# george-gca/sr-pytorch-lightning

Hardware: AMD Instinct MI355X
Metric: SR training throughput, LR patches/s (48x48 LR x4, fwd+bwd+Adam) (higher is better)
Workload: dtype bf16; 1 GPU; edsr_baseline x4, 48x48 LR patches, batch 256/GPU, train step (L1 + Adam); global_batch=256, parallelism=dp1, hip_graph=full

## Files before the change

### include/srk.h

```cpp
#ifndef SRK_H
#define SRK_H

#include <stdint.h>

#ifdef __cplusplus
extern "C" {
#endif

typedef void* srk_stream_t;

enum { SRK_BF16 = 0, SRK_F16 = 1, SRK_F32 = 2 };

enum {
  SRK_E_BADARG = -1,
  SRK_E_NODEV = -2
};

enum {
  SRK_OUT_NHWC = 0,
  SRK_OUT_NHWC_PS = 1,
  SRK_OUT_PLANAR = 2
};

typedef struct {
// ... 171 lines not shown
} srk_unfold_args;
int srk_unfold_nchw(const srk_unfold_args* a, srk_stream_t stream);

typedef struct {
  const float* src; void* dst; int dst_pitch, dst_coff;
  int N, C, H, W;
  int Cstore; int ps_r; float scale; int dtype;
} srk_to_nhwc_args;
int srk_nchw_to_nhwc(const srk_to_nhwc_args* a, srk_stream_t stream);

typedef struct {
  const void* src; int src_pitch, src_coff; float* dst;
  int N, C, H, W; int dtype;
} srk_to_nchw_args;
int srk_nhwc_to_nchw(const srk_to_nchw_args* a, srk_stream_t stream);

int srk_ca_splits(int N, int HW);
typedef struct {
  const void* t; int t_pitch, t_coff;
  const void* u; int u_pitch, u_coff;
  float* sums;
  int N, HW, C; int dtype;
} srk_ca_pool_args;
int srk_ca_pool(const srk_ca_pool_args* a, srk_stream_t stream);

typedef struct {
  const void* t; int t_pitch, t_coff;
  const void* res; int res_pitch, res_coff;
  const float* sums;
  const float* w1; const float* b1; const float* w2; const float* b2;
  float* s_out; float* z_out;
  void* out; int out_pitch, out_coff;
  int N, HW, C, Cr; int dtype;
  int sums_rows;
} srk_ca_apply_args;
int srk_ca_apply(const srk_ca_apply_args* a, srk_stream_t stream);

typedef struct {
  const void* g; int g_pitch, g_coff;
  const float* gsum;
  const float* sums; const float* s; const float* z;
  const float* w1; const float* w2;
  float* dw1; float* db1; float* dw2; float* db2;
  void* gt; int gt_pitch, gt_coff;
  int N, HW, C, Cr; int dtype;
  int sums_rows, gsum_rows;
} srk_ca_bwd_args;
int srk_ca_bwd_apply(const srk_ca_bwd_args* a, srk_stream_t stream);
typedef struct { const float* src; float* dst; int n; int k; } srk_rowsum_job;
int srk_rowsum_group(const srk_rowsum_job* table_dev, int njobs, int max_k, srk_stream_t stream);

typedef struct {
  const uint8_t* lr; const uint8_t* hr;
  int lr_h, lr_w, hr_h, hr_w;
  int top, left;
  int rot;
  int hflip, vflip;
} srk_patch_desc;
typedef struct {
  const srk_patch_desc* table; int N; int C; int patch_lr; int scale;
  float* lr_out;
  float* hr_out;
} srk_patch_args;
int srk_sample_patches(const srk_patch_args* a, srk_stream_t stream);

typedef struct {
  const float* sr; const float* hr;
  int N, C, H, W;
  int luma;
  int shave;
  double* sse;
} srk_sse_args;
int srk_image_sse(const srk_sse_args* a, srk_stream_t stream);

typedef struct srk_l1_args {
  const float* sr;
  const float* hr;
  long long n;
  signed char* sign;
  double* partial;
  const float* gout;
  float scale;
  float* grad;
} srk_l1_args;
int srk_l1_blocks(long long n);
int srk_l1_loss_fwd(const srk_l1_args* a, srk_stream_t stream);
int srk_l1_loss_bwd(const srk_l1_args* a, srk_stream_t stream);
int srk_l1_loss_mean(const double* partial, int nb, long long n, float* out, srk_stream_t stream);

#define SRK_FLIP_TABLE_FLOATS 176
#define SRK_FLIP_ADJ_CHANNELS 7
typedef struct srk_flip_args {
  const float* sr;
  const float* hr;
  int N, H, W;
  const float* table;
  double* partial;
  float* err;
  float* adj;
  const float* gout;
  float scale;
  float* grad;
} srk_flip_args;
int srk_flip_blocks(int N, int H, int W);
int srk_flip_fwd(const srk_flip_args* a, srk_stream_t stream);
int srk_flip_bwd(const srk_flip_args* a, srk_stream_t stream);
int srk_flip_mean(const double* partial, int nb, long long n, float* out, srk_stream_t stream);

typedef struct srk_haarpsi_args {
  const float* sr;
  const float* hr;
  int N, C, H, W;
  double* partial;
  float* planes;
  float* stats;
  float* loss;
  float* index;
  const float* gout;
  float* grad;
} srk_haarpsi_args;
int srk_haarpsi_tiles(int N, int H, int W);
int srk_haarpsi_fwd(const srk_haarpsi_args* a, srk_stream_t stream);
int srk_haarpsi_finalize(const srk_haarpsi_args* a, srk_stream_t stream);
int srk_haarpsi_bwd(const srk_haarpsi_args* a, srk_stream_t stream);

typedef struct srk_ssim_args {
  const float* x;
  const float* y;
  int N, C, H, W;
  int pool;
  float sigma, k1, k2;
  double* sums;
} srk_ssim_args;
int srk_image_ssim(const srk_ssim_args* a, srk_stream_t stream);

typedef struct srk_ms_ssim_args {
  const float* x;
  const float* y;
  float* workspace;
  double* partials;
  float* out;
  int N, C, H, W;
  float sigma, k1, k2;
  float w0, w1, w2, w3, w4;
} srk_ms_ssim_args;
long long srk_ms_ssim_workspace_bytes(int N, int C, int H, int W);
int srk_ms_ssim_tiles(int H, int W, int* first);
int srk_ms_ssim(const srk_ms_ssim_args* a, srk_stream_t stream);

typedef struct {
  const void* x; int x_pitch, x_coff;
  void* cols; int cols_pitch;
  int N, H, W, C;
  int K, stride, pad;
  int Ho, Wo;
  int dtype;
} srk_unfold_nhwc_args;
int srk_unfold_nhwc(const srk_unfold_nhwc_args* a, srk_stream_t stream);

typedef struct {
  const void* cols; int cols_pitch;
  const float* bias;
  void* out; int out_pitch, out_coff;
  int N, Hi, Wi, C;
  int K, stride, pad;
  int Ho, Wo;
  int dtype;
} srk_fold_nhwc_args;
int srk_fold_nhwc(const srk_fold_nhwc_args* a, srk_stream_t stream);

// ... 160 lines not shown
```

### sr-pytorch-lightning_amd/_lib.py

```python
import ctypes as C
import os

_HERE = os.path.dirname(os.path.abspath(__file__))
EXACT_RELU = os.environ.get("SRK_EXACT_RELU") == "1"
LIB_PATH = os.environ.get("SRK_LIB_PATH") or os.path.join(_HERE, "libsrk_gfx950_exact.so" if EXACT_RELU else "libsrk_gfx950.so")

SRK_BF16, SRK_F16, SRK_F32 = 0, 1, 2
OUT_NHWC, OUT_NHWC_PS, OUT_PLANAR = 0, 1, 2

_p, _i, _f = C.c_void_p, C.c_int, C.c_float


class PackArgs(C.Structure):
    _fields_ = [("w", _p), ("bias", _p), ("wpk", _p), ("bias_pk", _p),
                ("Cout", _i), ("Cin", _i), ("KH", _i), ("KW", _i),
                ("KinP", _i), ("CoutP", _i), ("dgrad", _i), ("ps_r", _i), ("dtype", _i), ("rows_layout", _i)]


class ConvArgs(C.Structure):
    _fields_ = [("x", _p), ("x_pitch", _i), ("x_coff", _i), ("x_ps", _i),
                ("N", _i), ("H", _i), ("W", _i), ("Cin", _i),
                ("wpk", _p), ("bias", _p), ("CoutP", _i), ("Cout", _i), ("KH", _i), ("KW", _i),
                ("relu", _i), ("scale", _f),
                ("res", _p), ("res_pitch", _i), ("res_coff", _i),
# ... 96 lines not shown
                ("N", _i), ("H", _i), ("W", _i), ("Cin", _i), ("Cout", _i), ("KH", _i), ("KW", _i),
                ("dwp", _p), ("dbp", _p), ("nslabs", _i), ("dtype", _i), ("cout_real", _i)]


class WgradFinArgs(C.Structure):
    _fields_ = [("dwp", _p), ("dbp", _p), ("nslabs", _i), ("dw", _p), ("db", _p),
                ("Cout", _i), ("Cin", _i), ("KH", _i), ("KW", _i), ("CinP", _i), ("CoutP", _i),
                ("ps_r", _i), ("scale", _f), ("accumulate", _i)]


class ProjArgs(C.Structure):
    _fields_ = [("x", _p), ("x_pitch", _i), ("out", _p), ("out_pitch", _i), ("wpk", _p), ("bias", _p),
                ("N", _i), ("H", _i), ("W", _i), ("dtype", _i), ("slope", _p), ("slope_stride", _i), ("pre", _p), ("pre_pitch", _i)]


class ProjPackJob(C.Structure):
    _fields_ = [("w4", _p), ("wpk", _p)]


class ProjWgradArgs(C.Structure):
    _fields_ = [("xh", _p), ("xh_pitch", _i), ("g", _p), ("g_pitch", _i), ("scratch", _p), ("dw", _p), ("accumulate", _i),
                ("N", _i), ("H", _i), ("W", _i), ("dtype", _i), ("db", _p), ("bias_side", _i), ("db_accumulate", _i)]


class UnfoldArgs(C.Structure):
    _fields_ = [("x", _p), ("sub", _p), ("dst", _p), ("dst_pitch", _i), ("dst_coff", _i),
                ("N", _i), ("Cin", _i), ("H", _i), ("W", _i), ("KH", _i), ("KW", _i), ("Kstore", _i), ("dtype", _i)]


class ToNhwcArgs(C.Structure):
    _fields_ = [("src", _p), ("dst", _p), ("dst_pitch", _i), ("dst_coff", _i),
                ("N", _i), ("C", _i), ("H", _i), ("W", _i), ("Cstore", _i), ("ps_r", _i), ("scale", _f), ("dtype", _i)]


class ToNchwArgs(C.Structure):
    _fields_ = [("src", _p), ("src_pitch", _i), ("src_coff", _i), ("dst", _p),
                ("N", _i), ("C", _i), ("H", _i), ("W", _i), ("dtype", _i)]


class CaPoolArgs(C.Structure):
    _fields_ = [("t", _p), ("t_pitch", _i), ("t_coff", _i), ("u", _p), ("u_pitch", _i), ("u_coff", _i),
                ("sums", _p), ("N", _i), ("HW", _i), ("C", _i), ("dtype", _i)]


class CaApplyArgs(C.Structure):
    _fields_ = [("t", _p), ("t_pitch", _i), ("t_coff", _i), ("res", _p), ("res_pitch", _i), ("res_coff", _i),
                ("sums", _p), ("w1", _p), ("b1", _p), ("w2", _p), ("b2", _p), ("s_out", _p), ("z_out", _p),
                ("out", _p), ("out_pitch", _i), ("out_coff", _i),
                ("N", _i), ("HW", _i), ("C", _i), ("Cr", _i), ("dtype", _i), ("sums_rows", _i)]


class CaBwdArgs(C.Structure):
    _fields_ = [("g", _p), ("g_pitch", _i), ("g_coff", _i), ("gsum", _p), ("sums", _p), ("s", _p), ("z", _p),
                ("w1", _p), ("w2", _p), ("dw1", _p), ("db1", _p), ("dw2", _p), ("db2", _p),
                ("gt", _p), ("gt_pitch", _i), ("gt_coff", _i),
                ("N", _i), ("HW", _i), ("C", _i), ("Cr", _i), ("dtype", _i), ("sums_rows", _i), ("gsum_rows", _i)]


class PatchDesc(C.Structure):
    _fields_ = [("lr", _p), ("hr", _p), ("lr_h", _i), ("lr_w", _i), ("hr_h", _i), ("hr_w", _i),
                ("top", _i), ("left", _i), ("rot", _i), ("hflip", _i), ("vflip", _i)]


class PatchArgs(C.Structure):
    _fields_ = [("table", _p), ("N", _i), ("C", _i), ("patch_lr", _i), ("scale", _i), ("lr_out", _p), ("hr_out", _p)]


class SseArgs(C.Structure):
    _fields_ = [("sr", _p), ("hr", _p), ("N", _i), ("C", _i), ("H", _i), ("W", _i), ("luma", _i), ("shave", _i), ("sse", _p)]


class SsimArgs(C.Structure):
    _fields_ = [("x", _p), ("y", _p), ("N", _i), ("C", _i), ("H", _i), ("W", _i), ("pool", _i),
                ("sigma", _f), ("k1", _f), ("k2", _f), ("sums", _p)]


class MsSsimArgs(C.Structure):
    _fields_ = [("x", _p), ("y", _p), ("workspace", _p), ("partials", _p), ("out", _p), ("N", _i), ("C", _i), ("H", _i), ("W", _i),
                ("sigma", _f), ("k1", _f), ("k2", _f), ("w0", _f), ("w1", _f), ("w2", _f), ("w3", _f), ("w4", _f)]


class L1Args(C.Structure):
    _fields_ = [("sr", _p), ("hr", _p), ("n", C.c_longlong), ("sign", _p), ("partial", _p), ("gout", _p),
                ("scale", _f), ("grad", _p)]


class FlipArgs(C.Structure):
    _fields_ = [("sr", _p), ("hr", _p), ("N", _i), ("H", _i), ("W", _i), ("table", _p), ("partial", _p), ("err", _p), ("adj", _p),
                ("gout", _p), ("scale", _f), ("grad", _p)]


class HaarpsiArgs(C.Structure):
    _fields_ = [("sr", _p), ("hr", _p), ("N", _i), ("C", _i), ("H", _i), ("W", _i), ("partial", _p), ("planes", _p), ("stats", _p), ("loss", _p),
                ("index", _p), ("gout", _p), ("grad", _p)]


class UnfoldNhwcArgs(C.Structure):
    _fields_ = [("x", _p), ("x_pitch", _i), ("x_coff", _i), ("cols", _p), ("cols_pitch", _i),
                ("N", _i), ("H", _i), ("W", _i), ("C", _i), ("K", _i), ("stride", _i), ("pad", _i), ("Ho", _i), ("Wo", _i), ("dtype", _i)]


class FoldNhwcArgs(C.Structure):
    _fields_ = [("cols", _p), ("cols_pitch", _i), ("bias", _p), ("out", _p), ("out_pitch", _i), ("out_coff", _i),
                ("N", _i), ("Hi", _i), ("Wi", _i), ("C", _i), ("K", _i), ("stride", _i), ("pad", _i), ("Ho", _i), ("Wo", _i), ("dtype", _i)]


class ChanStatsArgs(C.Structure):
    _fields_ = [("x", _p), ("x_pitch", _i), ("x_coff", _i), ("y", _p), ("y_pitch", _i), ("y_coff", _i),
                ("P", C.c_longlong), ("C", _i), ("mode", _i), ("partial", _p), ("dtype", _i), ("shift", _p), ("shift_out", _p),
                ("gate_out", _p), ("gate_pitch", _i), ("slope", _p), ("slope_stride", _i),
                ("gate_a", _p), ("gate_d", _p), ("partial2", _p)]


class ChanApplyArgs(C.Structure):
    _fields_ = [("x", _p), ("x_pitch", _i), ("x_coff", _i), ("y", _p), ("y_pitch", _i), ("y_coff", _i),
                ("z", _p), ("z_pitch", _i), ("z_coff", _i), ("a", _p), ("b", _p), ("d", _p),
                ("slope", _p), ("slope_stride", _i), ("post_prelu", _i), ("out", _p), ("out_pitch", _i), ("out_coff", _i),
                ("P", C.c_longlong), ("C", _i), ("dtype", _i), ("gate_a", _p), ("gate_d", _p)]


class HrTailArgs(C.Structure):
    _fields_ = [("wt", _p), ("bt", _p), ("wu", _p), ("bu", _p), ("O", _i), ("C", _i), ("Ci", _i),
                ("weff", _p), ("beff", _p), ("wedge", _p), ("bedge", _p), ("wcor", _p), ("bcor", _p),
                ("x", _p), ("x_pitch", _i), ("N", _i), ("H", _i), ("W", _i), ("dtype", _i),
                ("out", _p), ("g", _p), ("dx", _p), ("dx_pitch", _i),
                ("eedge", _p), ("e0", _p), ("ecor", _p), ("k0", _p), ("scratch", _p),
                ("r", _p), ("r0", _p), ("dwt", _p), ("dbt", _p), ("dwu", _p), ("dbu", _p)]


LAUNCHERS = {
    "srk_pack_conv_weights": PackArgs,
    "srk_conv2d": ConvArgs,
    "srk_conv_pair": ConvPairArgs,
    "srk_pw_pack": PwPackArgs,
    "srk_pw_forward": PwArgs,
    "srk_pw_backward": PwBwdArgs,
    "srk_pw_wgrad": PwWgradArgs,
    "srk_adam_step": AdamArgs,
    "srk_ranger_step": RangerArgs,
    "srk_sgd_step": SgdArgs,
    "srk_rmsprop_step": RmspropArgs,
    "srk_chan_finalize": ChanFinalizeArgs,
    "srk_conv2d_wgrad": WgradArgs,
    "srk_wgrad_finalize": WgradFinArgs,
    "srk_unfold_nchw": UnfoldArgs,
    "srk_nchw_to_nhwc": ToNhwcArgs,
    "srk_nhwc_to_nchw": ToNchwArgs,
    "srk_ca_pool": CaPoolArgs,
    "srk_ca_apply": CaApplyArgs,
    "srk_ca_bwd_apply": CaBwdArgs,
    "srk_sample_patches": PatchArgs,
    "srk_image_sse": SseArgs,
    "srk_image_ssim": SsimArgs,
    "srk_ms_ssim": MsSsimArgs,
    "srk_l1_loss_fwd": L1Args,
    "srk_l1_loss_bwd": L1Args,
    "srk_flip_fwd": FlipArgs,
    "srk_flip_bwd": FlipArgs,
    "srk_haarpsi_fwd": HaarpsiArgs,
    "srk_haarpsi_finalize": HaarpsiArgs,
    "srk_haarpsi_bwd": HaarpsiArgs,
    "srk_unfold_nhwc": UnfoldNhwcArgs,
    "srk_fold_nhwc": FoldNhwcArgs,
    "srk_chan_stats": ChanStatsArgs,
    "srk_chan_apply": ChanApplyArgs,
    "srk_proj_down": ProjArgs,
    "srk_proj_up": ProjArgs,
    "srk_proj_wgrad": ProjWgradArgs,
    "srk_hrtail_collapse": HrTailArgs,
    "srk_hrtail_edge_fwd": HrTailArgs,
    "srk_hrtail_edge_bwd_x": HrTailArgs,
    "srk_hrtail_edge_bwd_w": HrTailArgs,
    "srk_hrtail_expand": HrTailArgs,
}
OTHER_SYMBOLS = ("srk_conv_tile", "srk_last_error", "srk_version", "srk_device_cus", "srk_wgrad_slabs",
                 "srk_pack_conv_weights_group", "srk_l1_blocks", "srk_wgrad_group_ok", "srk_wgrad_group_job_bytes",
                 "srk_wgrad_group_plan", "srk_conv2d_wgrad_group", "srk_wgrad_finalize_group", "srk_upload_small", "srk_upload_prepare", "srk_upload_eager", "srk_upload_fence", "srk_ca_splits", "srk_chan_stats_blocks",
                 "srk_conv_pair_tiles", "srk_rowsum_group", "srk_pw_shape_ok", "srk_pw_pack_bytes", "srk_pw_pack_group", "srk_weight_norm_group", "srk_pw_wgrad_ranges", "srk_l1_loss_mean", "srk_chan_stats_finalize", "srk_pack_group_tiles", "srk_pack_conv_weights_group_tiled",
                 "srk_proj_pack", "srk_proj_pack_bytes", "srk_proj_wgrad_scratch_floats", "srk_proj_pack_group", "srk_wgrad_slab_cout",
                 "srk_hrtail_scratch_floats", "srk_adam_step_scaled", "srk_adam_check_scaled", "srk_adam_update_scaled", "srk_loss_scale_update", "srk_conv_bits_ok",
                 "srk_ranger_step_scaled", "srk_ranger_check_scaled", "srk_ranger_update_scaled",
                 "srk_sgd_step_scaled", "srk_sgd_check_scaled", "srk_sgd_update_scaled",
                 "srk_rmsprop_step_scaled", "srk_rmsprop_check_scaled", "srk_rmsprop_update_scaled",
                 "srk_conv_trunk", "srk_conv_trunk_ok", "srk_flip_blocks", "srk_flip_mean",
                 "srk_ms_ssim_workspace_bytes", "srk_ms_ssim_tiles", "srk_haarpsi_tiles")

_lib = None


def load():
    global _lib
    if _lib is not None:
        return _lib
    if not os.path.exists(LIB_PATH):
        raise RuntimeError(
            f"{LIB_PATH} is missing: build it with `python __graft_entry__.py` "
            "(hipcc --offload-arch=gfx950).  There is no CPU fallback for the HIP path.")
    lib = C.CDLL(LIB_PATH)
    older = bool(os.environ.get("SRK_LIB_PATH"))

    class _Absent:
        def __init__(self, name):
            self.name = name
            self.argtypes = self.restype = None

        def __call__(self, *a, **k):
            raise RuntimeError(f"{self.name} is not exported by {LIB_PATH} (an older build loaded through SRK_LIB_PATH)")

    if older:
        for name in list(LAUNCHERS) + list(OTHER_SYMBOLS):
            if not hasattr(lib, name):
                setattr(lib, name, _Absent(name))
    for name, st in LAUNCHERS.items():
        fn = getattr(lib, name)
        fn.argtypes = [C.POINTER(st), C.c_void_p]
        fn.restype = C.c_int
    lib.srk_conv_tile.argtypes = [C.c_int]
    lib.srk_conv_tile.restype = C.c_int
    lib.srk_conv_pair_tiles.argtypes = [C.c_int, C.c_int, C.c_int]
    lib.srk_conv_pair_tiles.restype = C.c_int
    lib.srk_wgrad_slabs.argtypes = [C.POINTER(WgradArgs)]
    lib.srk_wgrad_slabs.restype = C.c_int
    lib.srk_wgrad_slab_cout.argtypes = [C.POINTER(WgradArgs)]
    lib.srk_wgrad_slab_cout.restype = C.c_int
    lib.srk_pack_conv_weights_group.argtypes = [C.c_void_p, C.c_int, C.c_void_p]
    lib.srk_pack_conv_weights_group.restype = C.c_int
    lib.srk_pack_group_tiles.argtypes = [C.c_void_p, C.c_int, C.c_void_p]
    lib.srk_pack_group_tiles.restype = C.c_int
    lib.srk_pack_conv_weights_group_tiled.argtypes = [C.c_void_p, C.c_void_p, C.c_int, C.c_int, C.c_void_p]
    lib.srk_pack_conv_weights_group_tiled.restype = C.c_int
    lib.srk_wgrad_group_ok.argtypes = [C.POINTER(WgradArgs)]
    lib.srk_wgrad_group_ok.restype = C.c_int
    lib.srk_wgrad_group_job_bytes.restype = C.c_int
    lib.srk_wgrad_group_plan.argtypes = [C.POINTER(WgradArgs), C.c_int, C.c_void_p, C.c_void_p, C.c_void_p,
                                         C.POINTER(C.c_int), C.POINTER(C.c_longlong)]
    lib.srk_wgrad_group_plan.restype = C.c_int
    lib.srk_conv2d_wgrad_group.argtypes = [C.c_void_p, C.c_void_p, C.c_int, C.c_int, C.c_void_p]
    lib.srk_conv2d_wgrad_group.restype = C.c_int
    lib.srk_wgrad_finalize_group.argtypes = [C.c_void_p, C.c_int, C.c_int, C.c_void_p]
# ... 100 lines not shown
```

### sr-pytorch-lightning_amd/csrc/data.hip

```cpp
#include "srk_common.h"

namespace {

__device__ __forceinline__ void src_of(int y, int x, int S, int rot, int hf, int vf, int& i, int& j) {
  if (vf) y = S - 1 - y;
  if (hf) x = S - 1 - x;
  switch (rot & 3) {
    case 0: i = y; j = x; break;
    case 1: i = x; j = S - 1 - y; break;
    case 2: i = S - 1 - y; j = S - 1 - x; break;
    default: i = S - 1 - x; j = y; break;
  }
}

__global__ __launch_bounds__(256) void patch_kernel(const srk_patch_args a) {
  const int n = blockIdx.y;
  const srk_patch_desc d = a.table[n];
  const int pl = a.patch_lr, ph = a.patch_lr * a.scale;
  const int npl = pl * pl, nph = ph * ph;
  for (int t = blockIdx.x * blockDim.x + threadIdx.x; t < npl + nph; t += gridDim.x * blockDim.x) {
    const bool is_hr = t >= npl;
    const int q = is_hr ? t - npl : t;
    const int S = is_hr ? ph : pl;
    const int y = q / S, x = q - y * S;
// ... 100 lines not shown
    float m[5] = {0.f, 0.f, 0.f, 0.f, 0.f};
#pragma unroll
    for (int k = 0; k < 11; ++k) {
      const float w = g[k];
#pragma unroll
      for (int q = 0; q < 5; ++q) m[q] += w * Hm[q][r + k][c];
    }
    const float c1 = a.k1 * a.k1, c2 = a.k2 * a.k2;
    const float sxx = m[2] - m[0] * m[0], syy = m[3] - m[1] * m[1], sxy = m[4] - m[0] * m[1];
    const float cs = (2.f * sxy + c2) / (sxx + syy + c2);
    const float ss = (2.f * m[0] * m[1] + c1) / (m[0] * m[0] + m[1] * m[1] + c1) * cs;
    acc = (double)ss;
  }
#pragma unroll
  for (int off = 32; off > 0; off >>= 1) acc += __shfl_down(acc, off, 64);
  if ((tid & 63) == 0) red[tid >> 6] = acc;
  __syncthreads();
  if (tid == 0) atomicAdd(a.sums + plane, red[0] + red[1] + red[2] + red[3]);
}

constexpr int L1_BLOCKS_MAX = 2048;
__global__ __launch_bounds__(256) void l1_fwd_kernel(const srk_l1_args a) {
  __shared__ double red[4];
  const long long n4 = a.n >> 2;
  double acc = 0.0;
  for (long long i = (long long)blockIdx.x * 256 + threadIdx.x; i < n4; i += (long long)gridDim.x * 256) {
    const float4 s = reinterpret_cast<const float4*>(a.sr)[i], h = reinterpret_cast<const float4*>(a.hr)[i];
    const float d[4] = {s.x - h.x, s.y - h.y, s.z - h.z, s.w - h.w};
    unsigned pk = 0;
    float t = 0.f;
#pragma unroll
    for (int k = 0; k < 4; ++k) {
      t += fabsf(d[k]);
      const int sg = (d[k] > 0.f) - (d[k] < 0.f);
      pk |= (unsigned)(sg & 0xff) << (8 * k);
    }
    acc += (double)t;
    reinterpret_cast<unsigned*>(a.sign)[i] = pk;
  }
  if (blockIdx.x == 0 && threadIdx.x < (a.n & 3)) {
    const long long i = (n4 << 2) + threadIdx.x;
    const float d = a.sr[i] - a.hr[i];
    acc += (double)fabsf(d);
    a.sign[i] = (signed char)((d > 0.f) - (d < 0.f));
  }
#pragma unroll
  for (int off = 32; off > 0; off >>= 1) acc += __shfl_down(acc, off, 64);
  if ((threadIdx.x & 63) == 0) red[threadIdx.x >> 6] = acc;
  __syncthreads();
  if (threadIdx.x == 0) a.partial[blockIdx.x] = red[0] + red[1] + red[2] + red[3];
}
__global__ __launch_bounds__(64) void l1_mean_kernel(const double* __restrict__ partial, int nb, long long n, float* __restrict__ out) {
  double t = 0.0;
  int i = threadIdx.x;
  for (; i + 64 * 7 < nb; i += 64 * 8) {
    double v[8];
#pragma unroll
    for (int k = 0; k < 8; ++k) v[k] = partial[i + 64 * k];
#pragma unroll
    for (int k = 0; k < 8; ++k) t += v[k];
  }
  for (; i < nb; i += 64) t += partial[i];
#pragma unroll
  for (int off = 32; off > 0; off >>= 1) t += __shfl_down(t, off, 64);
  if (threadIdx.x == 0) *out = (float)(t / (double)n);
}
__global__ __launch_bounds__(256) void l1_bwd_kernel(const srk_l1_args a) {
  const float g = *a.gout * a.scale;
  const long long n4 = a.n >> 2;
  for (long long i = (long long)blockIdx.x * 256 + threadIdx.x; i < n4; i += (long long)gridDim.x * 256) {
    const unsigned pk = reinterpret_cast<const unsigned*>(a.sign)[i];
    float4 o;
    o.x = g * (float)(signed char)(pk & 0xff);
    o.y = g * (float)(signed char)((pk >> 8) & 0xff);
    o.z = g * (float)(signed char)((pk >> 16) & 0xff);
    o.w = g * (float)(signed char)(pk >> 24);
    reinterpret_cast<float4*>(a.grad)[i] = o;
  }
  if (blockIdx.x == 0 && threadIdx.x < (a.n & 3)) {
    const long long i = (n4 << 2) + threadIdx.x;
    a.grad[i] = g * (float)a.sign[i];
  }
}

}

extern "C" int srk_l1_blocks(long long n) {
  const long long b = (n / 4 + 255) / 256;
  return (int)(b < 1 ? 1 : (b > L1_BLOCKS_MAX ? L1_BLOCKS_MAX : b));
}
extern "C" int srk_l1_loss_fwd(const srk_l1_args* a, srk_stream_t stream) {
  SRK_CHECK_ARG(a && a->sr && a->hr && a->sign && a->partial && a->n > 0, "srk_l1_loss_fwd: null pointer / empty");
  SRK_CHECK_ARG(((uintptr_t)a->sr | (uintptr_t)a->hr | (uintptr_t)a->sign) % 16 == 0, "srk_l1_loss_fwd: 16-byte alignment");
  hipLaunchKernelGGL(l1_fwd_kernel, dim3(srk_l1_blocks(a->n)), dim3(256), 0, reinterpret_cast<hipStream_t>(stream), *a);
  SRK_LAUNCH_CHECK();
  return 0;
}
extern "C" int srk_l1_loss_mean(const double* partial, int nb, long long n, float* out, srk_stream_t stream) {
  SRK_CHECK_ARG(partial && out && nb > 0 && n > 0, "srk_l1_loss_mean: null pointer / empty");
  hipLaunchKernelGGL(l1_mean_kernel, dim3(1), dim3(64), 0, reinterpret_cast<hipStream_t>(stream), partial, nb, n, out);
  SRK_LAUNCH_CHECK();
  return 0;
}
extern "C" int srk_l1_loss_bwd(const srk_l1_args* a, srk_stream_t stream) {
  SRK_CHECK_ARG(a && a->sign && a->gout && a->grad && a->n > 0, "srk_l1_loss_bwd: null pointer / empty");
  SRK_CHECK_ARG(((uintptr_t)a->grad | (uintptr_t)a->sign) % 16 == 0, "srk_l1_loss_bwd: 16-byte alignment");
  hipLaunchKernelGGL(l1_bwd_kernel, dim3(srk_l1_blocks(a->n)), dim3(256), 0, reinterpret_cast<hipStream_t>(stream), *a);
  SRK_LAUNCH_CHECK();
  return 0;
}

extern "C" int srk_image_ssim(const srk_ssim_args* a, srk_stream_t stream) {
  SRK_CHECK_ARG(a && a->x && a->y && a->sums, "srk_image_ssim: null pointer");
  SRK_CHECK_ARG(a->N > 0 && a->C > 0 && (long long)a->N * a->C <= 65535 && a->pool >= 1 && a->sigma > 0.f, "srk_image_ssim: bad sizes");
  const int Hp = a->H / a->pool, Wp = a->W / a->pool;
  SRK_CHECK_ARG(Hp >= 11 && Wp >= 11, "srk_image_ssim: image %dx%d (pooled %dx%d) is smaller than the 11x11 window", a->H, a->W, Hp, Wp);
  const int tilesX = (Wp - 10 + 15) / 16, tilesY = (Hp - 10 + 15) / 16;
  hipLaunchKernelGGL(ssim_kernel, dim3((unsigned)(tilesX * tilesY), (unsigned)(a->N * a->C)), dim3(256), 0,
                     reinterpret_cast<hipStream_t>(stream), *a, tilesX, Hp, Wp);
  SRK_LAUNCH_CHECK();
  return 0;
}

extern "C" int srk_sample_patches(const srk_patch_args* a, srk_stream_t stream) {
  SRK_CHECK_ARG(a && a->table && a->lr_out && a->hr_out, "srk_sample_patches: null pointer");
  SRK_CHECK_ARG(a->N > 0 && a->N <= 65535 && a->C > 0 && a->C <= 4 && a->patch_lr > 0 && a->scale > 0, "srk_sample_patches: bad sizes");
  const int total = a->patch_lr * a->patch_lr * (1 + a->scale * a->scale);
  int gx = (total + 255) / 256;
  if (gx > 64) gx = 64;
  hipLaunchKernelGGL(patch_kernel, dim3(gx, a->N), dim3(256), 0, reinterpret_cast<hipStream_t>(stream), *a);
  SRK_LAUNCH_CHECK();
  return 0;
}

extern "C" int srk_image_sse(const srk_sse_args* a, srk_stream_t stream) {
  SRK_CHECK_ARG(a && a->sr && a->hr && a->sse, "srk_image_sse: null pointer");
  SRK_CHECK_ARG(a->N > 0 && a->N <= 65535 && a->C > 0 && a->H > 2 * a->shave && a->W > 2 * a->shave && a->shave >= 0, "srk_image_sse: bad sizes");
  SRK_CHECK_ARG(!a->luma || a->C == 3, "srk_image_sse: luma needs 3 channels");
  const long long npix = (long long)(a->H - 2 * a->shave) * (a->W - 2 * a->shave);
  long long gx = (npix + 255) / 256;
  if (gx > 512) gx = 512;
  hipLaunchKernelGGL(sse_kernel, dim3((unsigned)gx, a->N), dim3(256), 0, reinterpret_cast<hipStream_t>(stream), *a);
  SRK_LAUNCH_CHECK();
  return 0;
}
```

### sr-pytorch-lightning_amd/ops.py

```python
import weakref

import torch

from . import _lib as L
from .packing import *
from .packing import _DT, _TLS, _f32c, _group_for, _knob, _need_gpu, _ptr, _roundup, _stream, _tok


def _pitch(t):
    n, h, w, c = t.shape
    p = t.stride(2) if w > 1 else (t.stride(1) if h > 1 else (t.stride(0) if n > 1 else c))
    if w > 1 and h > 1:
        assert t.stride(1) == w * p, "NHWC view must be dense in W"
    if h > 1 and n > 1:
        assert t.stride(0) == h * w * p, "NHWC view must be dense in H"
    assert c == 1 or t.stride(3) == 1, "channels must be innermost"
    return p


_ADDR_LIMIT = 0x7fff0000


def _batch_chunks(n, *tensors):
    worst = 0
# ... 346 lines not shown

    @staticmethod
    def forward(ctx, x, w, b, sub, ps_r, dtype):
        _need_gpu(x)
        cout, cin, k, _ = w.shape
        n, c, h, wd = x.shape
        r = ps_r if ps_r > 1 else 1
        xu = unfold_raw(x, sub, k, dtype)
        pk = _pack_head(w, b, dtype)
        out = torch.empty((n, cout // (r * r), h * r, wd * r), dtype=torch.float32, device=x.device)
        conv_raw(xu, pk, N=n, H=h, W=wd, Cin=xu.shape[3], Cout=cout, out=out, out_mode=L.OUT_PLANAR, ps_r=ps_r)
        ctx.save_for_backward(xu, w)
        ctx.cfg = (ps_r, b is not None)
        return out

    @staticmethod
    def backward(ctx, g):
        xu, w = ctx.saved_tensors
        ps_r, has_b = ctx.cfg
        n, h, wd, kp = xu.shape
        gw = gb = None
        if ctx.needs_input_grad[1] or ctx.needs_input_grad[2]:
            dy = to_nhwc(g, xu.dtype, ps_r=ps_r)
            gw, gb = wgrad_raw(xu, dy, N=n, H=h, W=wd, Cin=kp, Cout=dy.shape[3], k=1, w_shape=tuple(w.shape),
                               want_bias=has_b)
            gw = gw if ctx.needs_input_grad[1] else None
        return None, gw, gb, None, None, None


def skip_conv(x, w, b, sub, ps_r, dtype):
    return SkipConvFn.apply(x, w, b, sub, int(ps_r), dtype)


_HR_COLLAPSE = _knob("SRK_NO_HR_COLLAPSE", "0") != "1"


def hr_tail_ok(x, wu, wt, ps_r):
    if not _HR_COLLAPSE or int(ps_r) != 2 or x.dtype not in (torch.bfloat16, torch.float16):
        return False
    cu, ci, ku, _ = wu.shape
    o, c, kt, _ = wt.shape
    if ku != 3 or kt != 3 or cu != 4 * c or ci != 64 or x.shape[3] != 64 or not 1 <= o <= 4:
        return False
    n, h, w, _ = x.shape
    return n > 0 and max(h, w) <= 512 and x.numel() * 2 < _ADDR_LIMIT and n * o * 4 * h * w < (1 << 31)


def _hr_bufs(o, ci, dev):
    f32 = torch.float32
    return dict(weff=torch.empty((4 * o, ci, 5, 5), dtype=f32, device=dev), beff=torch.empty(4 * o, dtype=f32, device=dev),
                wedge=torch.empty((4, 2 * o, ci, 5), dtype=f32, device=dev), bedge=torch.empty((4, 2 * o), dtype=f32, device=dev),
                wcor=torch.empty((4, o, ci), dtype=f32, device=dev), bcor=torch.empty((4, o), dtype=f32, device=dev))


class HrTailFn(torch.autograd.Function):

    @staticmethod
    def _args(x, wu, bu, wt, bt, bufs, **kw):
        n, h, w, _ = x.shape
        o, c = wt.shape[0], wt.shape[1]
        return L.HrTailArgs(wt=wt.data_ptr(), bt=_ptr(bt), wu=wu.data_ptr(), bu=_ptr(bu), O=o, C=c, Ci=wu.shape[1],
                            weff=bufs["weff"].data_ptr(), beff=bufs["beff"].data_ptr(), wedge=bufs["wedge"].data_ptr(),
                            bedge=bufs["bedge"].data_ptr(), wcor=bufs["wcor"].data_ptr(), bcor=bufs["bcor"].data_ptr(),
                            x=x.data_ptr(), x_pitch=_pitch(x), N=n, H=h, W=w, dtype=_DT[x.dtype], **kw)

    @staticmethod
    def forward(ctx, x, wu, bu, wt, bt, post_add):
        _need_gpu(x)
        n, h, w, ci = x.shape
        o = wt.shape[0]
        dev, f32 = x.device, torch.float32
        wu_, wt_ = _f32c(wu), _f32c(wt)
        bu_, bt_ = (None if bu is None else _f32c(bu)), (None if bt is None else _f32c(bt))
        bufs = _hr_bufs(o, ci, dev)
        L.call("srk_hrtail_collapse", HrTailFn._args(x, wu_, bu_, wt_, bt_, bufs), _stream())
        pk = pack_conv(bufs["weff"], bufs["beff"], x.dtype, cache=False)
        out = torch.empty((n, o, 2 * h, 2 * w), dtype=f32, device=dev)
        conv_raw(x, pk, N=n, H=h, W=w, Cin=ci, Cout=4 * o, out=out, out_mode=L.OUT_PLANAR, ps_r=2, post_add=post_add)
        L.call("srk_hrtail_edge_fwd", HrTailFn._args(x, wu_, bu_, wt_, bt_, bufs, out=out.data_ptr()), _stream())
        ctx.save_for_backward(x, wu_, wt_, *( [bu_] if bu_ is not None else []))
        ctx.has = (bu is not None, bt is not None)
        ctx.bufs = bufs
        ctx.wb = (wu, bu, wt, bt)
        return out

    @staticmethod
    def backward(ctx, g):
        x, wu_, wt_ = ctx.saved_tensors[:3]
        has_bu, has_bt = ctx.has
        bu_ = ctx.saved_tensors[3] if has_bu else None
        bufs = ctx.bufs
        n, h, w, ci = x.shape
        o, c = wt_.shape[0], wt_.shape[1]
        dev, f32 = x.device, torch.float32
        g = _f32c(g)
        st = _stream()
        g12 = to_nhwc(g, x.dtype, ps_r=2)
        need_x = ctx.needs_input_grad[0]
        need_w = any(ctx.needs_input_grad[1:5])
        gx = None
        if need_x:
            pkd = pack_conv(bufs["weff"], None, x.dtype, dgrad=True, cache=False)
            gx = torch.empty_like(x)
            conv_raw(g12, pkd, N=n, H=h, W=w, Cin=g12.shape[3], Cout=ci, out=gx, use_bias=False)
            L.call("srk_hrtail_edge_bwd_x", HrTailFn._args(x, wu_, bu_, wt_, None, bufs, g=g.data_ptr(), dx=gx.data_ptr(), dx_pitch=_pitch(gx)), st)
        gwu = gbu = gwt = gbt = None
        if need_w:
            r, r0 = wgrad_raw(x, g12, N=n, H=h, W=w, Cin=ci, Cout=g12.shape[3], k=5, w_shape=(4 * o, ci, 5, 5), want_bias=True)
            red = dict(eedge=torch.empty((4, 2 * o, ci, 5), dtype=f32, device=dev), e0=torch.empty((4, 2 * o), dtype=f32, device=dev),
                       ecor=torch.empty((4, o, ci), dtype=f32, device=dev), k0=torch.empty((4, o), dtype=f32, device=dev))
            scratch = torch.empty(int(L.load().srk_hrtail_scratch_floats(n, ci)), dtype=f32, device=dev)
            ptrs = {k: v.data_ptr() for k, v in red.items()}
            L.call("srk_hrtail_edge_bwd_w", HrTailFn._args(x, wu_, bu_, wt_, None, bufs, g=g.data_ptr(), scratch=scratch.data_ptr(), **ptrs), st)
            pu, pbu, pt, pbt = ctx.wb
            gwu, gwt = (route(p, shape, dev, slice=p.dtype == f32, buffer=True).out for p, shape in ((pu, tuple(wu_.shape)), (pt, tuple(wt_.shape))))
            gbu = route(pbu, (4 * c,), dev, slice=pbu.dtype == f32, buffer=True).out if has_bu else None
            gbt = route(pbt, (o,), dev, slice=pbt.dtype == f32, buffer=True).out if has_bt else None
            L.call("srk_hrtail_expand", HrTailFn._args(x, wu_, bu_, wt_, None, bufs, r=r.data_ptr(), r0=r0.data_ptr(), dwt=gwt.data_ptr(),
                                                       dbt=_ptr(gbt), dwu=gwu.data_ptr(), dbu=_ptr(gbu), **ptrs), st)
        return gx, gwu, gbu, gwt, gbt, None


def hr_tail(x, wu, bu, wt, bt, *, post_add=None):
    return HrTailFn.apply(x, wu, bu, wt, bt, post_add)


class ConvChainFn(torch.autograd.Function):

    @staticmethod
    def forward(ctx, x, scale, relus, *params):
        _need_gpu(x)
        L_ = len(relus)
        ws, bs = params[0::2], params[1::2]
        n, h, wd, _ = x.shape
        acts = [x]
        bits = []
        a = x
        paired = L_ == 2 and tuple(relus) == (True, False) and pair_ok(x, ws[0], ws[1])
        if paired:
            y1 = torch.empty_like(x)
            a = conv_pair_raw(x, pack_conv(ws[0], bs[0], x.dtype), pack_conv(ws[1], bs[1], x.dtype), out=torch.empty_like(x),
                              relu_mid=True, mid=y1, scale_out=scale, res=x)
            acts.append(y1)
        for i in range(0 if paired else L_):
            w = ws[i]
            cout, cin, k, _ = w.shape
            pk = pack_conv(w, bs[i], x.dtype)
            out = torch.empty((n, h, wd, pad16(cout)), dtype=x.dtype, device=x.device)
            last = i == L_ - 1
            conv_raw(a, pk, N=n, H=h, W=wd, Cin=a.shape[3], Cout=out.shape[3], out=out, relu=relus[i],
                     scale=scale if last else 1.0, res=x if last else None,
                     relu_bits="want" if (relus[i] and not last and ctx.needs_input_grad[0]) else None)
            a = out
            if not last:
                acts.append(a)
                bits.append(out.__dict__.pop("_srk_bits", None))
        ctx.bits = bits
        ctx.save_for_backward(*acts, *ws)
        ctx.cfg = (scale, tuple(relus), tuple(b is not None for b in bs))
        ctx.wb = (tuple(ws), tuple(bs))
        ctx.pg = _tok()
        return a

    @staticmethod
    def backward(ctx, g):
        scale, relus, has_b = ctx.cfg
        L_ = len(relus)
        acts, ws = ctx.saved_tensors[:L_], ctx.saved_tensors[L_:]
        g = g.contiguous()
        n, h, wd, _ = g.shape
        grads = [None] * (2 * L_)
        dy = g
        paired = L_ == 2 and relus == (True, False) and pair_ok(g, ws[0], ws[1])
        if paired:
            x, y1 = acts
            g1 = torch.empty_like(g)
            gx = conv_pair_raw(g, pack_conv(ws[1], None, g.dtype, dgrad=True, token=ctx.pg),
                               pack_conv(ws[0], None, g.dtype, dgrad=True, token=ctx.pg), out=torch.empty_like(g),
                               scale_mid=scale, mask=y1, mid=g1, res=g, use_bias=False)
            for i, (a_in, d, sc) in enumerate(((x, g1, 1.0), (y1, g, scale))):
# ... 751 lines not shown
```

### sr-pytorch-lightning_amd/ops_metrics.py

```python
import ctypes
import os

import torch

from . import _lib as L
from .ops import _f32c, _need_gpu, _stream


def image_sse(sr, hr, *, luma=False, shave=0):
    _need_gpu(sr)
    n, c, h, w = sr.shape
    s32, h32 = _f32c(sr), _f32c(hr)
    sse = torch.zeros(n, dtype=torch.float64, device=sr.device)
    a = L.SseArgs(sr=s32.data_ptr(), hr=h32.data_ptr(), N=n, C=c, H=h, W=w, luma=int(luma), shave=int(shave), sse=sse.data_ptr())
    L.call("srk_image_sse", a, _stream())
    count = (h - 2 * shave) * (w - 2 * shave) * (1 if luma else c)
    return sse, count


def psnr(sr, hr, *, luma=False, shave=0, eps=1e-8):
    sse, count = image_sse(sr, hr, luma=luma, shave=shave)
    return (10.0 * torch.log10(1.0 / (sse / count + eps))).mean().float()


def ssim(x, y, *, sigma=1.5, k1=0.01, k2=0.03):
    _need_gpu(x)
    xs, ys = _f32c(x), _f32c(y)
    n, c, h, w = xs.shape
    f = max(1, round(min(h, w) / 256))
    sums = torch.zeros(n * c, dtype=torch.float64, device=xs.device)
    a = L.SsimArgs(x=xs.data_ptr(), y=ys.data_ptr(), N=n, C=c, H=h, W=w, pool=f, sigma=float(sigma), k1=float(k1), k2=float(k2),
                   sums=sums.data_ptr())
    L.call("srk_image_ssim", a, _stream())
    count = (h // f - 10) * (w // f - 10)
    return (sums / count).mean().float()


MS_SSIM_WEIGHTS = (0.0448, 0.2856, 0.3001, 0.2363, 0.1333)
MS_SSIM_MIN_SIZE = (11 - 1) * 2 ** (len(MS_SSIM_WEIGHTS) - 1) + 1


def ms_ssim_check(x, y):
    if x.dim() != 4 or tuple(x.shape) != tuple(y.shape):
        raise ValueError(f"ms_ssim expects two N x C x H x W tensors of one shape, got {tuple(x.shape)} and {tuple(y.shape)}")
    if min(x.shape[-2:]) < MS_SSIM_MIN_SIZE:
        raise ValueError(f"Invalid size of the input images, expected at least {MS_SSIM_MIN_SIZE}x{MS_SSIM_MIN_SIZE}.")


def _ms_ssim_launch(x, y, sigma, k1, k2):
    _need_gpu(x)
    ms_ssim_check(x, y)
    xs, ys = _f32c(x), _f32c(y)
    n, c, h, w = xs.shape
    lib = L.load()
    first = (ctypes.c_int * (len(MS_SSIM_WEIGHTS) + 1))()
    tiles = lib.srk_ms_ssim_tiles(h, w, first)
    pyr = lib.srk_ms_ssim_workspace_bytes(n, c, h, w)
    if tiles <= 0 or pyr < 0:
        raise RuntimeError(f"srk_ms_ssim refused the sizes {tuple(xs.shape)}")
    ws = torch.empty(pyr + n * c * tiles * 16, dtype=torch.uint8, device=xs.device)
    out = torch.empty((), dtype=torch.float32, device=xs.device)
    w0, w1, w2, w3, w4 = MS_SSIM_WEIGHTS
    a = L.MsSsimArgs(x=xs.data_ptr(), y=ys.data_ptr(), workspace=ws.data_ptr(), partials=ws.data_ptr() + pyr, out=out.data_ptr(),
                     N=n, C=c, H=h, W=w, sigma=float(sigma), k1=float(k1), k2=float(k2), w0=w0, w1=w1, w2=w2, w3=w3, w4=w4)
    L.call("srk_ms_ssim", a, _stream())
    return out, ws[pyr:].view(torch.float64).view(n * c, tiles, 2), list(first)


def ms_ssim(x, y, *, sigma=1.5, k1=0.01, k2=0.03):
    return _ms_ssim_launch(x, y, sigma, k1, k2)[0]


def ms_ssim_levels(x, y, *, sigma=1.5, k1=0.01, k2=0.03):
    out, part, first = _ms_ssim_launch(x, y, sigma, k1, k2)
    n, c, h, w = x.shape
    hs, ws = [h], [w]
    for _ in range(len(MS_SSIM_WEIGHTS) - 1):
        p = max(hs[-1] % 2, ws[-1] % 2)
        hs.append((hs[-1] + p) // 2)
        ws.append((ws[-1] + p) // 2)
    cs, ss = [], []
    for k in range(len(MS_SSIM_WEIGHTS)):
        s = part[:, first[k]:first[k + 1]].sum(dim=1) / ((hs[k] - 10) * (ws[k] - 10))
        ss.append(s[:, 0].view(n, c))
        cs.append(s[:, 1].view(n, c))
    return out, torch.stack(cs), torch.stack(ss)


class L1LossFn(torch.autograd.Function):

    @staticmethod
    def forward(ctx, sr, hr):
        _need_gpu(sr)
        s, h = _f32c(sr), _f32c(hr)
        n = s.numel()
        sign = torch.empty(n, dtype=torch.int8, device=s.device)
        nb = L.load().srk_l1_blocks(n)
        partial = torch.empty(nb, dtype=torch.float64, device=s.device)
        a = L.L1Args(sr=s.data_ptr(), hr=h.data_ptr(), n=n, sign=sign.data_ptr(), partial=partial.data_ptr(), gout=0, scale=0.0, grad=0)
        L.call("srk_l1_loss_fwd", a, _stream())
        ctx.save_for_backward(sign)
        ctx.shape = tuple(sr.shape)
        out = torch.empty((), dtype=torch.float32, device=s.device)
        L.check(L.load().srk_l1_loss_mean(partial.data_ptr(), nb, n, out.data_ptr(), _stream()), "srk_l1_loss_mean")
        return out

    @staticmethod
    def backward(ctx, g):
        (sign,) = ctx.saved_tensors
        n = sign.numel()
        gout = g.detach().float().contiguous()
        grad = torch.empty(ctx.shape, dtype=torch.float32, device=sign.device)
        a = L.L1Args(sr=0, hr=0, n=n, sign=sign.data_ptr(), partial=0, gout=gout.data_ptr(), scale=1.0 / n, grad=grad.data_ptr())
        L.call("srk_l1_loss_bwd", a, _stream())
        return grad, None


def l1_loss(sr, hr):
    if hr.requires_grad or sr.numel() == 0:
        return torch.nn.functional.l1_loss(sr, hr)
    return L1LossFn.apply(sr, hr)
```

Measured before the change: 47980 LR patches/s.

## Fuse L1 loss backward with pixel-shuffle NHWC repack of the HR-tail gradient

The L1 backward kernel now also writes the gradient directly in the 16-bit pixel-unshuffled NHWC layout that the HR-tail backward needs. The tensors are tagged through __dict__, so the HR-tail backward can reuse that buffer and skip its separate to_nhwc conversion pass over the fp32 gradient. This removes one full read of the HR-resolution gradient and one kernel launch. The cost is cross-op coupling through tensor attributes, version checks and weakrefs, plus guards for hooks and retained grads.

Result: no change. 48210 LR patches/s (median of 6 runs) (+0.5%).

```diff
diff --git a/include/srk.h b/include/srk.h
--- a/include/srk.h
+++ b/include/srk.h
@@ -277,10 +277,14 @@
   const float* gout;
   float scale;
   float* grad;
+  void* g12;
+  int B, O, H, W;
+  int dtype;
 } srk_l1_args;
 int srk_l1_blocks(long long n);
 int srk_l1_loss_fwd(const srk_l1_args* a, srk_stream_t stream);
 int srk_l1_loss_bwd(const srk_l1_args* a, srk_stream_t stream);
+int srk_l1_loss_bwd_ps(const srk_l1_args* a, srk_stream_t stream);
 int srk_l1_loss_mean(const double* partial, int nb, long long n, float* out, srk_stream_t stream);
 
 #define SRK_FLIP_TABLE_FLOATS 176
diff --git a/sr-pytorch-lightning_amd/_lib.py b/sr-pytorch-lightning_amd/_lib.py
--- a/sr-pytorch-lightning_amd/_lib.py
+++ b/sr-pytorch-lightning_amd/_lib.py
@@ -202,7 +202,7 @@
 
 class L1Args(C.Structure):
     _fields_ = [("sr", _p), ("hr", _p), ("n", C.c_longlong), ("sign", _p), ("partial", _p), ("gout", _p),
-                ("scale", _f), ("grad", _p)]
+                ("scale", _f), ("grad", _p), ("g12", _p), ("B", _i), ("O", _i), ("H", _i), ("W", _i), ("dtype", _i)]
 
 
 class FlipArgs(C.Structure):
@@ -275,6 +275,7 @@
     "srk_ms_ssim": MsSsimArgs,
     "srk_l1_loss_fwd": L1Args,
     "srk_l1_loss_bwd": L1Args,
+    "srk_l1_loss_bwd_ps": L1Args,
     "srk_flip_fwd": FlipArgs,
     "srk_flip_bwd": FlipArgs,
     "srk_haarpsi_fwd": HaarpsiArgs,
diff --git a/sr-pytorch-lightning_amd/csrc/data.hip b/sr-pytorch-lightning_amd/csrc/data.hip
--- a/sr-pytorch-lightning_amd/csrc/data.hip
+++ b/sr-pytorch-lightning_amd/csrc/data.hip
@@ -206,6 +206,62 @@
     a.grad[i] = g * (float)a.sign[i];
   }
 }
+template <int DT, int PX> __global__ __launch_bounds__(256) void l1_bwd_ps_kernel(const srk_l1_args a) {
+  typedef DTraits<DT> Tr;
+  static_assert(Tr::IS16, "16-bit storage");
+  const float g = *a.gout * a.scale;
+  const int H = a.H, W = a.W, O = a.O, W2 = 2 * W, Wq = W / PX;
+  const size_t plane = (size_t)4 * H * W;
+  const long long total = (long long)a.B * H * Wq;
+  typename Tr::elem* const dst = reinterpret_cast<typename Tr::elem*>(a.g12);
+  for (long long t = (long long)blockIdx.x * 256 + threadIdx.x; t < total; t += (long long)gridDim.x * 256) {
+    const int x = (int)(t % Wq) * PX;
+    const long long q = t / Wq;
+    const int y = (int)(q % H), n = (int)(q / H);
+    float v[PX][16];
+#pragma unroll
+    for (int px = 0; px < PX; ++px)
+#pragma unroll
+      for (int c = 0; c < 16; ++c) v[px][c] = 0.f;
+#pragma unroll
+    for (int o = 0; o < 4; ++o) {
+      if (o >= O) break;
+#pragma unroll
+      for (int r = 0; r < 2; ++r) {
+        const size_t at = (size_t)(n * O + o) * plane + (size_t)(2 * y + r) * W2 + 2 * x;
+        if constexpr (PX == 2) {
+          const unsigned pk = *reinterpret_cast<const unsigned*>(a.sign + at);
+          f32x4 f;
+          f.x = g * (float)(signed char)(pk & 0xff);
+          f.y = g * (float)(signed char)((pk >> 8) & 0xff);
+          f.z = g * (float)(signed char)((pk >> 16) & 0xff);
+          f.w = g * (float)(signed char)(pk >> 24);
+          *reinterpret_cast<f32x4*>(a.grad + at) = f;
+          v[0][o * 4 + r * 2] = f.x; v[0][o * 4 + r * 2 + 1] = f.y;
+          v[1][o * 4 + r * 2] = f.z; v[1][o * 4 + r * 2 + 1] = f.w;
+        } else {
+          const unsigned pk = *reinterpret_cast<const unsigned short*>(a.sign + at);
+          float2 f;
+          f.x = g * (float)(signed char)(pk & 0xff);
+          f.y = g * (float)(signed char)(pk >> 8);
+          *reinterpret_cast<float2*>(a.grad + at) = f;
+          v[0][o * 4 + r * 2] = f.x; v[0][o * 4 + r * 2 + 1] = f.y;
+        }
+      }
+    }
+#pragma unroll
+    for (int px = 0; px < PX; ++px) {
+      typename Tr::elem* const d = dst + ((size_t)(n * H + y) * W + x + px) * 16;
+#pragma unroll
+      for (int h = 0; h < 2; ++h) {
+        i32x4 raw;
+        raw.x = (int)pack2<DT>(v[px][8 * h + 0], v[px][8 * h + 1]); raw.y = (int)pack2<DT>(v[px][8 * h + 2], v[px][8 * h + 3]);
+        raw.z = (int)pack2<DT>(v[px][8 * h + 4], v[px][8 * h + 5]); raw.w = (int)pack2<DT>(v[px][8 * h + 6], v[px][8 * h + 7]);
+        *reinterpret_cast<i32x4*>(d + 8 * h) = raw;
+      }
+    }
+  }
+}
 
 }
 
@@ -230,6 +286,28 @@
   SRK_CHECK_ARG(a && a->sign && a->gout && a->grad && a->n > 0, "srk_l1_loss_bwd: null pointer / empty");
   SRK_CHECK_ARG(((uintptr_t)a->grad | (uintptr_t)a->sign) % 16 == 0, "srk_l1_loss_bwd: 16-byte alignment");
   hipLaunchKernelGGL(l1_bwd_kernel, dim3(srk_l1_blocks(a->n)), dim3(256), 0, reinterpret_cast<hipStream_t>(stream), *a);
+  SRK_LAUNCH_CHECK();
+  return 0;
+}
+
+extern "C" int srk_l1_loss_bwd_ps(const srk_l1_args* a, srk_stream_t stream) {
+  SRK_CHECK_ARG(a && a->sign && a->gout && a->grad && a->g12, "srk_l1_loss_bwd_ps: null pointer");
+  SRK_CHECK_ARG(a->B > 0 && a->H > 0 && a->W > 0 && a->O >= 1 && a->O <= 4 && a->n == (long long)a->B * a->O * 4 * a->H * a->W &&
+                (long long)a->B * a->O < (1ll << 31) && (long long)a->B * a->H < (1ll << 31),
+                "srk_l1_loss_bwd_ps: n=%lld for B=%d O=%d (<= 4) H=%d W=%d", a->n, a->B, a->O, a->H, a->W);
+  SRK_CHECK_ARG(a->dtype == SRK_BF16 || a->dtype == SRK_F16, "srk_l1_loss_bwd_ps: dtype %d (16-bit storage only)", a->dtype);
+  SRK_CHECK_ARG(((uintptr_t)a->grad | (uintptr_t)a->sign | (uintptr_t)a->g12) % 16 == 0, "srk_l1_loss_bwd_ps: 16-byte alignment");
+  hipStream_t st = reinterpret_cast<hipStream_t>(stream);
+  const bool two = a->W % 2 == 0;
+  const long long lanes = (long long)a->B * a->H * (two ? a->W / 2 : a->W);
+  const dim3 grid((unsigned)((lanes + 255) / 256 > 16384 ? 16384 : (lanes + 255) / 256));
+  if (a->dtype == SRK_BF16) {
+    if (two) hipLaunchKernelGGL((l1_bwd_ps_kernel<SRK_BF16, 2>), grid, dim3(256), 0, st, *a);
+    else hipLaunchKernelGGL((l1_bwd_ps_kernel<SRK_BF16, 1>), grid, dim3(256), 0, st, *a);
+  } else {
+    if (two) hipLaunchKernelGGL((l1_bwd_ps_kernel<SRK_F16, 2>), grid, dim3(256), 0, st, *a);
+    else hipLaunchKernelGGL((l1_bwd_ps_kernel<SRK_F16, 1>), grid, dim3(256), 0, st, *a);
+  }
   SRK_LAUNCH_CHECK();
   return 0;
 }
diff --git a/sr-pytorch-lightning_amd/ops.py b/sr-pytorch-lightning_amd/ops.py
--- a/sr-pytorch-lightning_amd/ops.py
+++ b/sr-pytorch-lightning_amd/ops.py
@@ -452,6 +452,8 @@
         ctx.has = (bu is not None, bt is not None)
         ctx.bufs = bufs
         ctx.wb = (wu, bu, wt, bt)
+        out.__dict__["_srk_hrtail"] = (n, o, h, w, x.dtype)
+        ctx.out_ref = weakref.ref(out)
         return out
 
     @staticmethod
@@ -463,9 +465,18 @@
         n, h, w, ci = x.shape
         o, c = wt_.shape[0], wt_.shape[1]
         dev, f32 = x.device, torch.float32
+        made = g.__dict__.get("_srk_g12")
+        g12 = None
+        sr = ctx.out_ref()
+        if sr is not None and (sr._backward_hooks or sr.retains_grad):
+            made = None
+        if made is not None and made[1] == g._version and g.dtype == f32 and g.is_contiguous() and made[0].dtype == x.dtype \
+                and tuple(made[0].shape) == (n, h, w, 16) and tuple(g.shape) == (n, o, 2 * h, 2 * w):
+            g12 = made[0]
         g = _f32c(g)
         st = _stream()
-        g12 = to_nhwc(g, x.dtype, ps_r=2)
+        if g12 is None:
+            g12 = to_nhwc(g, x.dtype, ps_r=2)
         need_x = ctx.needs_input_grad[0]
         need_w = any(ctx.needs_input_grad[1:5])
         gx = None
diff --git a/sr-pytorch-lightning_amd/ops_metrics.py b/sr-pytorch-lightning_amd/ops_metrics.py
--- a/sr-pytorch-lightning_amd/ops_metrics.py
+++ b/sr-pytorch-lightning_amd/ops_metrics.py
@@ -4,7 +4,7 @@
 import torch
 
 from . import _lib as L
-from .ops import _f32c, _need_gpu, _stream
+from .ops import _DT, _f32c, _knob, _need_gpu, _stream
 
 
 def image_sse(sr, hr, *, luma=False, shave=0):
@@ -87,6 +87,9 @@
     return out, torch.stack(cs), torch.stack(ss)
 
 
+_FUSED_L1 = _knob("SRK_NO_FUSED_L1", "0") != "1"
+
+
 class L1LossFn(torch.autograd.Function):
 
     @staticmethod
@@ -101,6 +104,8 @@
         L.call("srk_l1_loss_fwd", a, _stream())
         ctx.save_for_backward(sign)
         ctx.shape = tuple(sr.shape)
+        tag = sr.__dict__.get("_srk_hrtail") if _FUSED_L1 else None
+        ctx.ps = tag if tag is not None and sr.dtype == torch.float32 and tuple(sr.shape) == (tag[0], tag[1], 2 * tag[2], 2 * tag[3]) else None
         out = torch.empty((), dtype=torch.float32, device=s.device)
         L.check(L.load().srk_l1_loss_mean(partial.data_ptr(), nb, n, out.data_ptr(), _stream()), "srk_l1_loss_mean")
         return out
@@ -111,6 +116,14 @@
         n = sign.numel()
         gout = g.detach().float().contiguous()
         grad = torch.empty(ctx.shape, dtype=torch.float32, device=sign.device)
+        if ctx.ps is not None:
+            b, o, h, w, dt = ctx.ps
+            g12 = torch.empty((b, h, w, 16), dtype=dt, device=sign.device)
+            a = L.L1Args(sr=0, hr=0, n=n, sign=sign.data_ptr(), partial=0, gout=gout.data_ptr(), scale=1.0 / n, grad=grad.data_ptr(),
+                         g12=g12.data_ptr(), B=b, O=o, H=h, W=w, dtype=_DT[dt])
+            L.call("srk_l1_loss_bwd_ps", a, _stream())
+            grad.__dict__["_srk_g12"] = (g12, grad._version)
+            return grad, None
         a = L.L1Args(sr=0, hr=0, n=n, sign=sign.data_ptr(), partial=0, gout=gout.data_ptr(), scale=1.0 / n, grad=grad.data_ptr())
         L.call("srk_l1_loss_bwd", a, _stream())
         return grad, None
```
